# baryshnikova-lab/safepy

Hardware: AMD Instinct MI355X
Metric: node-attribute enrichments/sec (nodes x attrs x perms), compute_pvalues permutation test (higher is better)
Workload: dtype u1 (bit-sliced integer counts; f64 outputs)

## Files before the change

### safepy_amd/csrc/attr.hip

```cpp
#include "common.h"

template <typename T>
__device__ __forceinline__ double load_attr(const void *raw, int64_t idx) {
    return static_cast<double>(reinterpret_cast<const T *>(raw)[idx]);
}

template <typename T, int GC>
__global__ __launch_bounds__(256) void k_attr_stats(const void *__restrict__ raw, int64_t n, int64_t m,
                                                    int64_t rs, int64_t cs, unsigned int *__restrict__ row_bits,
                                                    unsigned long long *__restrict__ acc ,
                                                    double *__restrict__ col_sum, unsigned long long *__restrict__ max_abs_bits,
                                                    unsigned int *__restrict__ col_nan, int64_t rows_per_block) {
    extern __shared__ unsigned int s_bits[];
    constexpr int RL = 256 / GC;
    const int cx = GC == 1 ? 0 : (threadIdx.x & (GC - 1));
    const int ry = GC == 1 ? threadIdx.x : (threadIdx.x / GC);
    const int lane = threadIdx.x & 63;
    const int64_t j = static_cast<int64_t>(blockIdx.x) * GC + cx;
    const int64_t n_words = (n + 31) / 32;
    __shared__ double s_sum[256];
    __shared__ double s_max[256];
    __shared__ unsigned int s_nan[256], s_other[256], s_nonint[256];
    const int64_t r_begin = static_cast<int64_t>(blockIdx.y) * rows_per_block;
    const int64_t r_end = r_begin + rows_per_block < n ? r_begin + rows_per_block : n;
    const int64_t w_begin = r_begin >> 5, w_end = (r_end + 31) >> 5;
    for (int64_t w = w_begin + threadIdx.x; w < w_end; w += 256) s_bits[w] = 0;
    __syncthreads();
    unsigned int c_nan = 0, c_other = 0, c_nonint = 0;
    double mx = 0.0, sum = 0.0;
    constexpr int UN = 4;
    const int64_t n_round = r_begin + (r_end - r_begin + UN * RL - 1) / (UN * RL) * (UN * RL);
    if (GC == 1 && rs == 1) {
        struct __attribute__((packed, aligned(sizeof(T)))) Vec { T v[4]; };
        const T *colp = static_cast<const T *>(raw) + j * cs;
        for (int64_t i0 = r_begin + 4 * static_cast<int64_t>(threadIdx.x); i0 < r_end; i0 += UN * 4 * 256) {
            Vec x[UN];
#pragma unroll
            for (int u = 0; u < UN; ++u) {
                const int64_t i = i0 + static_cast<int64_t>(u) * 4 * 256;
                if (i + 4 <= r_end) {
                    x[u] = *reinterpret_cast<const Vec *>(colp + i);
                } else {
#pragma unroll
                    for (int e = 0; e < 4; ++e) x[u].v[e] = i + e < r_end ? colp[i + e] : static_cast<T>(0);
                }
            }
#pragma unroll
            for (int u = 0; u < UN; ++u) {
                const int64_t i = i0 + static_cast<int64_t>(u) * 4 * 256;
                unsigned int nib = 0;
#pragma unroll
                for (int e = 0; e < 4; ++e) {
                    if (i + e >= r_end) continue;
                    const double v = static_cast<double>(x[u].v[e]);
                    if (v != v) {
                        ++c_nan;
                    } else {
                        nib |= 1u << e;
                        sum += v;
                        if (v != 0.0 && v != 1.0) ++c_other;
                        if (v != floor(v)) ++c_nonint;
                        const double a = fabs(v);
                        if (a > mx) mx = a;
                    }
                }
                if (nib) atomicOr(&s_bits[i >> 5], nib << (i & 31));
            }
        }
    } else
    for (int64_t i0 = r_begin + ry; i0 < n_round; i0 += UN * RL) {
        double v[UN];
        bool inb[UN];
#pragma unroll
        for (int u = 0; u < UN; ++u) {
            const int64_t i = i0 + u * RL;
            inb[u] = i < r_end && j < m;
            v[u] = inb[u] ? load_attr<T>(raw, i * rs + j * cs) : 0.0;
        }
#pragma unroll
        for (int u = 0; u < UN; ++u) {
            const int64_t i = i0 + u * RL;
            bool has = false;
            if (inb[u]) {
                if (v[u] != v[u]) {
                    ++c_nan;
                } else {
                    has = true;
                    sum += v[u];
                    if (v[u] != 0.0 && v[u] != 1.0) ++c_other;
                    if (v[u] != floor(v[u])) ++c_nonint;
                    const double a = fabs(v[u]);
                    if (a > mx) mx = a;
                }
            }
            const unsigned long long bal = __ballot(has);
            if (GC == 1) {
                const int64_t r0 = i - lane;
                if (lane == 0 && bal) {
                    if (r0 < r_end) s_bits[r0 >> 5] |= static_cast<unsigned int>(bal);
                    if (r0 + 32 < r_end) s_bits[(r0 >> 5) + 1] |= static_cast<unsigned int>(bal >> 32);
                }
            } else {
                if (lane == 0 && bal && i < r_end) atomicOr(&s_bits[i >> 5], 1u << (i & 31));
            }
        }
    }
    if (GC == 1) {
        for (int off = 32; off; off >>= 1) {
            sum += __shfl_down(sum, off);
            const double o = __shfl_down(mx, off);
            mx = o > mx ? o : mx;
            c_nan += __shfl_down(c_nan, off);
            c_other += __shfl_down(c_other, off);
            c_nonint += __shfl_down(c_nonint, off);
        }
    }
    const int slot = GC == 1 ? (lane == 0 ? static_cast<int>(threadIdx.x >> 6) : -1) : static_cast<int>(threadIdx.x);
    if (slot >= 0) {
        s_sum[slot] = sum;
        s_max[slot] = mx;
        s_nan[slot] = c_nan;
        s_other[slot] = c_other;
        s_nonint[slot] = c_nonint;
    }
    __syncthreads();
    for (int64_t w = w_begin + threadIdx.x; w < w_end; w += 256) {
        const unsigned int mine = s_bits[w];
        if (mine & ~row_bits[w]) atomicOr(&row_bits[w], mine);
    }
    if (ry == 0 && j < m) {
        double total = 0.0, tmx = 0.0;
        unsigned long long t_nan = 0, t_other = 0, t_nonint = 0;
        for (int r = 0; r < (GC == 1 ? 4 : RL); ++r) {
            const int t = GC == 1 ? r : r * GC + cx;
            total += s_sum[t];
            if (s_max[t] > tmx) tmx = s_max[t];
            t_nan += s_nan[t];
            t_other += s_other[t];
            t_nonint += s_nonint[t];
        }
        if (gridDim.y == 1) col_sum[j] = total;
        else atomicAdd(&col_sum[j], total);
        if (t_nan) atomicAdd(&col_nan[j], static_cast<unsigned int>(t_nan));
        if (t_other) atomicAdd(&acc[4 + (j & 63)], t_other);
        if (t_nonint) atomicAdd(&acc[68 + (j & 63)], t_nonint);
        const unsigned long long mine = static_cast<unsigned long long>(__double_as_longlong(tmx));
        if (mine > __builtin_nontemporal_load(max_abs_bits)) atomicMax(max_abs_bits, mine);
    }
}

__global__ __launch_bounds__(256) void k_stats_finish(unsigned long long *__restrict__ acc, const unsigned int *__restrict__ col_nan, int64_t m,
                                                      const unsigned int *__restrict__ bits, int64_t n, uint8_t *__restrict__ bytes,
                                                      unsigned long long *__restrict__ tail) {
    __shared__ unsigned int s_mx[4];
    __shared__ unsigned long long s_fold[2];
    unsigned int mx = 0;
    for (int64_t i = threadIdx.x; i < m; i += 256) mx = col_nan[i] > mx ? col_nan[i] : mx;
    for (int off = 32; off; off >>= 1) {
        const unsigned int o = __shfl_down(mx, off);
        mx = o > mx ? o : mx;
    }
    if ((threadIdx.x & 63) == 0) s_mx[threadIdx.x >> 6] = mx;
    if (threadIdx.x < 64) {
        unsigned long long a = acc[4 + threadIdx.x], b = acc[68 + threadIdx.x];
        for (int off = 32; off; off >>= 1) {
            a += __shfl_down(a, off);
            b += __shfl_down(b, off);
        }
        if (threadIdx.x == 0) s_fold[0] = a, s_fold[1] = b;
    }
    for (int64_t i = threadIdx.x; i < n; i += 256) bytes[i] = (bits[i >> 5] >> (i & 31)) & 1u;
    __syncthreads();
    if (threadIdx.x == 0) {
        const unsigned int m01 = s_mx[0] > s_mx[1] ? s_mx[0] : s_mx[1], m23 = s_mx[2] > s_mx[3] ? s_mx[2] : s_mx[3];
        tail[0] = acc[0] = s_fold[0];
        tail[1] = acc[1] = m01 > m23 ? m01 : m23;
        tail[2] = acc[2] = s_fold[1];
        tail[3] = acc[3];
    }
}

template <typename T>
__global__ __launch_bounds__(256) void k_fill_support(const void *__restrict__ raw, int64_t n, int64_t m, int64_t rs,
                                                      int64_t cs, const int32_t *__restrict__ sup_ptr,
                                                      int32_t *__restrict__ sup_row) {
    const int64_t j = (static_cast<int64_t>(blockIdx.x) * 256 + threadIdx.x) >> 6;
    const int lane = threadIdx.x & 63;
// ... 99 lines not shown
    SAFE_TRY(dev_alloc(&attr->sup_row, total));
    SAFE_HIP_CHECK(hipMemcpyAsync(attr->sup_ptr, attr->h_sup_ptr.data(), (m + 1) * sizeof(int32_t), hipMemcpyHostToDevice,
                                  ctx->stream));
    if (attr->dtype == SAFE_DTYPE_F32)
        hipLaunchKernelGGL(k_fill_support<float>, dim3(ceil_div(m * 64, 256)), dim3(256), 0, ctx->stream, attr->raw, n, m,
                           attr->row_stride, attr->col_stride, attr->sup_ptr, attr->sup_row);
    else
        hipLaunchKernelGGL(k_fill_support<double>, dim3(ceil_div(m * 64, 256)), dim3(256), 0, ctx->stream, attr->raw, n, m,
                           attr->row_stride, attr->col_stride, attr->sup_ptr, attr->sup_row);
    SAFE_HIP_CHECK(hipGetLastError());
    return SAFE_OK;
}

static size_t flags_block_bytes(int64_t n) { return static_cast<size_t>(ceil_div(n, 8)) * 8 + 32; }

int safe_attr_prepare(safe_attr *attr) {
    if (attr->stats_ready) return SAFE_OK;
    safe_ctx *ctx = attr->ctx;
    SAFE_HIP_CHECK(hipSetDevice(ctx->device));
    const int64_t n = attr->n, m = attr->m;
    const size_t flag_bytes = flags_block_bytes(n), tail_off = flag_bytes - 32;
    const int64_t n_words = (n + 31) / 32;
    SAFE_REQUIRE(n_words * sizeof(unsigned int) <= 150 * 1024, "safe_attr_stats: too many rows for the LDS row bitmap");
    void *tmp = nullptr;
    const size_t tmp_bytes = 132 * sizeof(unsigned long long) + static_cast<size_t>(n_words + m) * sizeof(unsigned int);
    SAFE_TRY(ctx_scratch(ctx, SCRATCH_ATTR_STATS, tmp_bytes, &tmp));
    unsigned long long *d_acc = static_cast<unsigned long long *>(tmp);
    unsigned int *d_rowbits = reinterpret_cast<unsigned int *>(d_acc + 132);
    unsigned int *d_colnan = d_rowbits + n_words;
    SAFE_HIP_CHECK(hipMemsetAsync(tmp, 0, tmp_bytes, ctx->stream));
    uint8_t *flags = nullptr;
    SAFE_TRY(ctx_block_alloc(ctx, flag_bytes, reinterpret_cast<void **>(&flags)));
    if (!attr->col_sum) SAFE_TRY(ctx_block_alloc(ctx, static_cast<size_t>(m) * sizeof(double), reinterpret_cast<void **>(&attr->col_sum)));
    const bool f32 = attr->dtype == SAFE_DTYPE_F32;
    const bool c_order = attr->col_stride == 1 && m > 1;
    if (c_order) SAFE_HIP_CHECK(hipMemsetAsync(attr->col_sum, 0, m * sizeof(double), ctx->stream));
#define STATS(T, GC, RPB)                                                                                          \
    do {                                                                                                           \
        if (n_words * sizeof(unsigned int) > 32 * 1024)                                                            \
            SAFE_HIP_CHECK(hipFuncSetAttribute(reinterpret_cast<const void *>(k_attr_stats<T, GC>),                \
                                               hipFuncAttributeMaxDynamicSharedMemorySize,                         \
                                               static_cast<int>(n_words * sizeof(unsigned int))));                 \
        hipLaunchKernelGGL((k_attr_stats<T, GC>), dim3(ceil_div(m, GC), ceil_div(n, RPB)), dim3(256),              \
                           n_words * sizeof(unsigned int), ctx->stream, attr->raw, n, m, attr->row_stride,         \
                           attr->col_stride, d_rowbits, d_acc, attr->col_sum, d_acc + 3, d_colnan,                 \
                           static_cast<int64_t>(RPB));                                                             \
    } while (0)
    if (c_order) {
        const int64_t groups = ceil_div(m, 64);
        const int64_t want_chunks = std::max<int64_t>(1, 2048 / groups);
        const int64_t rpb = std::max<int64_t>(256, ceil_div(ceil_div(n, want_chunks), 64) * 64);
        if (f32) STATS(float, 64, rpb);
        else STATS(double, 64, rpb);
    } else {
        if (f32) STATS(float, 1, n);
        else STATS(double, 1, n);
    }
#undef STATS
    hipLaunchKernelGGL(k_stats_finish, dim3(1), dim3(256), 0, ctx->stream, d_acc, d_colnan, m, d_rowbits, n, flags,
                       reinterpret_cast<unsigned long long *>(flags + tail_off));
    SAFE_HIP_CHECK(hipGetLastError());
    void *pinned = nullptr;
    SAFE_TRY(ctx_pinned(ctx, flag_bytes, &pinned));
    SAFE_HIP_CHECK(hipMemcpyAsync(pinned, flags, flag_bytes, hipMemcpyDeviceToHost, ctx->stream));
    SAFE_HIP_CHECK(safe_stream_sync(ctx->stream));
    const uint8_t *h_flags = static_cast<const uint8_t *>(pinned);
    unsigned long long h_acc[4];
    memcpy(h_acc, h_flags + tail_off, sizeof(h_acc));
    attr->n_other = static_cast<int64_t>(h_acc[0]);
    attr->max_nan_col = static_cast<int64_t>(h_acc[1]);
    attr->n_non_integer = static_cast<int64_t>(h_acc[2]);
    double mx;
    memcpy(&mx, &h_acc[3], sizeof(double));
    attr->max_abs = mx;
    if (!attr->flags_ready) {
        if (attr->row_flags) ctx_block_free(ctx, attr->row_flags, flag_bytes);
        attr->row_flags = flags;
        attr->flags_ready = true;
        int64_t cnt = 0;
        for (int64_t i = 0; i < n; ++i) cnt += h_flags[i] != 0;
        attr->n_rows_with_value = cnt;
        attr->h_row_flags.assign(h_flags, h_flags + n);
    } else {
        ctx_block_free(ctx, flags, flag_bytes);
    }
    attr->stats_ready = true;
    return SAFE_OK;
}

enum : unsigned int {
    CSC_PTR_FIRST = 1u,
    CSC_PTR_LAST = 2u,
    CSC_PTR_DECREASES = 4u,
    CSC_ROW_EQUAL = 8u,
    CSC_ROW_DESCENDS = 16u,
    CSC_ROW_RANGE = 32u,
    CSC_RULES = 63u,
    CSC_NOT_ONE = 256u,
    CSC_ON_MISSING = 512u,
};

template <typename T>
__global__ __launch_bounds__(256) void k_csc_validate(int64_t n, int64_t m, int64_t nnz, const int64_t *__restrict__ indptr,
                                                      const int32_t *__restrict__ indices, const T *__restrict__ values,
                                                      const uint8_t *__restrict__ missing, int32_t *__restrict__ sup_ptr,
                                                      unsigned int *__restrict__ flag) {
    const int64_t t = static_cast<int64_t>(blockIdx.x) * 256 + threadIdx.x;
    unsigned int bad = 0;
    if (t < nnz) {
        const int32_t r = indices[t];
        if (r < 0 || r >= n) bad |= CSC_ROW_RANGE;
// ... 414 lines not shown
```

### safepy_amd/csrc/common.h

```cpp
#pragma once
#include <hip/hip_runtime.h>

#include <algorithm>
#include <cstdarg>
#include <cmath>
#include <cstdint>
#include <cstdio>
#include <cstdlib>
#include <cstring>
#include <condition_variable>
#include <memory>
#include <mutex>
#include <atomic>
#include <string>
#include <thread>
#include <vector>

#include "safe_hip.h"
#include "bits_plan.h"

#define SAFE_WAVE 64
#define SAFE_PAD_U16 0xFFFFu

void safe_set_error(const char *fmt, ...);
// ... 232 lines not shown
    ~CallTimer() {
        for (hipEvent_t e : ev)
            if (e) (void)hipEventDestroy(e);
    }
    hipError_t start(hipStream_t s) {
        for (hipEvent_t &e : ev) {
            const hipError_t err = hipEventCreateWithFlags(&e, safe_event_flags(hipEventDefault));
            if (err != hipSuccess) return err;
        }
        return hipEventRecord(ev[0], s);
    }
    hipError_t stop(hipStream_t s) { return hipEventRecord(ev[1], s); }
    hipError_t ms(double *out) {
        float f = 0;
        const hipError_t err = hipEventElapsedTime(&f, ev[0], ev[1]);
        *out = f;
        return err;
    }
    hipError_t finish(safe_ctx *ctx, const char *name, int64_t launches, double *kernel_ms) {
        double t = 0;
        const hipError_t err = ms(&t);
        if (err != hipSuccess) return err;
        ctx->last_kernel.name = name;
        ctx->last_kernel.total_ms = ctx->last_kernel.busy_ms = t;
        ctx->last_kernel.launches = launches;
        ctx->last_kernel.summed = true;
        if (kernel_ms) *kernel_ms = t;
        return hipSuccess;
    }
};

struct safe_nbr {
    safe_ctx *ctx = nullptr;
    int64_t n = 0;
    int64_t nnz = 0;
    int64_t max_count = 0;
    int64_t words = 0;
    uint64_t *bits = nullptr;
    int32_t *row_ptr = nullptr;
    int32_t *col = nullptr;
    int64_t n_slices = 0;
    int32_t *sell_row = nullptr;
    int32_t *sell_pos = nullptr;
    int64_t *slice_off = nullptr;
    int32_t *slice_width = nullptr;
    int32_t *sell_col = nullptr;
    int64_t sell_entries = 0;
    uint16_t *sell_col2 = nullptr;
    uint16_t *sell_col2b = nullptr;
    std::vector<int32_t> h_slice_width;
    BitsTaskPlan bits_plan;
    void *bits_plan_pinned = nullptr;
    size_t bits_plan_pinned_bytes = 0;
    std::vector<int64_t> h_slice_off;
    std::vector<int32_t> h_row_count;
    double *dist = nullptr;
    int32_t *at_ptr = nullptr;
    int32_t *at_col = nullptr;
    std::vector<double> h_xy;
    bool blocks_ready = false;
    int64_t bs_groups = 0;
    int64_t bs_blocks = 0;
    int64_t bs_pieces = 0;
    int64_t bs_src = 0;
    int32_t *bs_order = nullptr;
    int32_t *bs_rowmap = nullptr;
    int32_t *bs_rowcnt = nullptr;
    int32_t *bs_grpmax = nullptr;
    uint4 *bs_bits4p = nullptr;
    int64_t bs_max_group_blocks = 0;
    int32_t *bs_ptr = nullptr;
    int32_t *bs_kb = nullptr;
    uint32_t *bs_bits = nullptr;
    std::vector<int32_t> h_bs_ptr;
    std::vector<int32_t> h_bs_rowmap;
    std::vector<int2> counts_tasks;
    int32_t counts_qoff[9] = {0};
    int64_t counts_tasks_grp = -1;
};

struct HypLookup {
    const int32_t *nid;
    const int32_t *kid;
    const double2 *tab;
    int64_t n_kid, xs;
    double p_cut;
    double *dummy;
    double *pvalues_pos, *nes, *nes_binary;
    unsigned int *enriched;
    unsigned int *cnt16;
    unsigned int *xmax;
    int dbg = 0;
};

static inline double nes_p_cut(double enrichment_threshold) {
    const double thr = -std::log10(enrichment_threshold);
    auto hit = [&](double p) { return -std::log10(p) > thr; };
    double p = enrichment_threshold;
    for (int it = 0; it < 4096 && hit(p); ++it) p = std::nextafter(p, 1.0);
    for (int it = 0; it < 4096 && !hit(std::nextafter(p, 0.0)); ++it) p = std::nextafter(p, 0.0);
    return p;
}

enum PermMode {
    PERM_SCORE = 0,
    PERM_COUNTS = 1,
// ... 147 lines not shown
```

### safepy_amd/csrc/enrich.hip

```cpp
#include <algorithm>
#include <cmath>
#include <numeric>

#include "common.h"
#include "hyp_math.h"

template <typename T, int BN, int PLANES>
__global__ __launch_bounds__(256) void k_tile_prep(const void *__restrict__ raw, int64_t n, int64_t rs, int64_t cs,
                                                   int64_t col0, int64_t mloc, int64_t n_tiles,
                                                   double *__restrict__ bt) {
    const int64_t idx = static_cast<int64_t>(blockIdx.x) * 256 + threadIdx.x;
    const int64_t total = n_tiles * (n + 1) * BN;
    if (idx >= total) return;
    const int c = static_cast<int>(idx % BN);
    const int64_t row = (idx / BN) % (n + 1);
    const int64_t tile = idx / (static_cast<int64_t>(BN) * (n + 1));
    const int64_t j = tile * BN + c;
    double v = 0.0, v2 = 0.0, nn = 0.0;
    if (row < n && j < mloc) {
        const T x = reinterpret_cast<const T *>(raw)[row * rs + (col0 + j) * cs];
        if (x == x) {
            v = static_cast<double>(x);
            v2 = static_cast<double>(static_cast<T>(x * x));
            nn = 1.0;
// ... 1116 lines not shown
            }
        } else {
            for (int p = 0; p < np; ++p) {
                uint32_t s0[LV], s1[LV];
#pragma unroll
                for (int l = 0; l < LV; ++l) s0[l] = s1[l] = 0;
                add_pairs(s0, s1);
                settle(p, s0, s1);
            }
        }
    } else {
        for (int p = 0; p < np; ++p, perm_ids += perm_stride) {
            uint32_t s0[LV], s1[LV];
            if (single) {
#pragma unroll
                for (int l = 0; l < LV; ++l) s0[l] = s1[l] = 0;
                const u32x4 *ahead = perm_ids + (p + 2 < np ? 2 * perm_stride : 0) + lane;
                if (p & 1) blk_add8<LV, 0, GATHER>(cb, ahead, s0, s1);
                else blk_add8<LV, 0, GATHER>(ca, ahead, s0, s1);
            } else
                blk_sum<LV, 0, GATHER, (DBG & 32) == 0>(perm_ids, lane, nblk, s0, s1);
            settle(p, s0, s1);
        }
    }
    vflush<CL>(g0, gp0);
    vflush<CL>(g1, gp1);
    vflush<CL>(l0, lp0);
    vflush<CL>(l1, lp1);
    if (STREAM) asm volatile("s_waitcnt vmcnt(0)" : : : "v112", "v113", "v114", "v115", "v116", "v117", "v118", "v119");
}
#pragma clang diagnostic pop

template <int LV, int CL, int DBG>
__device__ __forceinline__ void blk_task(const uint32_t *__restrict__ obs, const u32x4 *__restrict__ perm_ids, int64_t perm_stride,
                                         int lane, int nblk, int np, uint32_t (&g0)[CL], uint32_t (&g1)[CL], uint32_t (&l0)[CL],
                                         uint32_t (&l1)[CL]) {
    blk_task_core<LV, CL, DBG>(obs, perm_ids, perm_stride, lane, nblk, np, g0, g1, l0, l1);
}

template <int LV>
__device__ __forceinline__ void observed_wave(const u32x4 *__restrict__ ids, int lane, int nblk, uint32_t *__restrict__ obs,
                                              uint32_t (&oo0)[BT_LV], uint32_t (&oo1)[BT_LV]) {
    uint32_t o0[LV], o1[LV];
    blk_sum<LV, 2, 1>(ids, lane, nblk, o0, o1);
#pragma unroll
    for (int l = 0; l < BT_LV; ++l) {
        oo0[l] = l < LV ? o0[l < LV ? l : 0] : 0u;
        oo1[l] = l < LV ? o1[l < LV ? l : 0] : 0u;
        obs[l * 64 + lane] = oo0[l];
        obs[(BT_LV + l) * 64 + lane] = oo1[l];
    }
}

__global__ __launch_bounds__(256) void k_bits_observed(int64_t n, const int32_t *__restrict__ sell_row,
                                                       const int64_t *__restrict__ slice_off,
                                                       const int32_t *__restrict__ slice_width,
                                                       const uint16_t *__restrict__ sell_col2b, int64_t n_slices,
                                                       const uint2 *__restrict__ bbits, int64_t mloc,
                                                       uint32_t *__restrict__ obs, double *__restrict__ ns_out) {
    extern __shared__ unsigned int lds[];
    uint2 *T = reinterpret_cast<uint2 *>(lds);
    if ((uint32_t)(uintptr_t)((__attribute__((address_space(3))) unsigned int *)lds) != 0u) __builtin_trap();
    const int wave = __builtin_amdgcn_readfirstlane(threadIdx.x >> 6), lane = threadIdx.x & 63;
    const int64_t wg = blockIdx.x, s = static_cast<int64_t>(blockIdx.y) * 4 + wave;
    load_word_column(T, bbits + wg * (n + 1), n);
    __syncthreads();
    if (s >= n_slices) return;
    const int wdt = __builtin_amdgcn_readfirstlane(slice_width[s]);
    const u32x4 *ids = reinterpret_cast<const u32x4 *>(sell_col2b) + slice_off[s] / 8;
    uint32_t *my_obs = obs + (wg * n_slices + s) * (2 * BT_LV * 64);
    uint32_t oo0[BT_LV], oo1[BT_LV];
    if (wdt <= 8) observed_wave<4>(ids, lane, wdt >> 3, my_obs, oo0, oo1);
    else if (wdt <= 56) observed_wave<6>(ids, lane, wdt >> 3, my_obs, oo0, oo1);
    else if (wdt <= 248) observed_wave<8>(ids, lane, wdt >> 3, my_obs, oo0, oo1);
    else if (wdt <= 504) observed_wave<9>(ids, lane, wdt >> 3, my_obs, oo0, oo1);
    else observed_wave<BT_LV>(ids, lane, wdt >> 3, my_obs, oo0, oo1);
    if (ns_out) {
        const int32_t row = sell_row[s * 64 + lane];
        uint16_t *tile = reinterpret_cast<uint16_t *>(lds + 2 * ((n + 2) & ~int64_t(1)) + 4) + wave * (64 * 66);
#pragma unroll
        for (int half = 0; half < 2; ++half)
#pragma unroll
            for (int bit = 0; bit < 32; ++bit)
                tile[lane * 66 + half * 32 + bit] = static_cast<uint16_t>(half ? vextract<BT_LV>(oo1, bit) : vextract<BT_LV>(oo0, bit));
        const int64_t jc = wg * 64 + lane;
#pragma unroll 8
        for (int r = 0; r < 64; ++r) {
            const int32_t row_r = __shfl(row, r);
            if (row_r >= 0 && jc < mloc) ns_out[static_cast<int64_t>(row_r) * mloc + jc] = static_cast<double>(tile[r * 66 + lane]);
        }
    }
}

template <int CL, bool PLAIN_STORE = false>
__device__ __forceinline__ void flush_counters(const uint32_t (&g0)[CL], const uint32_t (&g1)[CL], const uint32_t (&l0)[CL],
                                               const uint32_t (&l1)[CL], unsigned int *__restrict__ gl_counts, int64_t col0,
                                               int64_t mloc, int64_t n_pad, int64_t spos, bool active) {
#pragma unroll
    for (int half = 0; half < 2; ++half) {
        uint32_t m[32];
#pragma unroll
        for (int l = 0; l < 16; ++l) {
            m[l] = l < CL ? (half ? g1[l < CL ? l : 0] : g0[l < CL ? l : 0]) : 0u;
            m[16 + l] = l < CL ? (half ? l1[l < CL ? l : 0] : l0[l < CL ? l : 0]) : 0u;
        }
        transpose32(m);
        const int64_t c_first = col0 + half * 32;
        const int n_valid = static_cast<int>(mloc - c_first < 32 ? (mloc - c_first > 0 ? mloc - c_first : 0) : 32);
        int64_t off = c_first * n_pad + spos;
#pragma unroll
        for (int bit = 0; bit < 32; ++bit) {
            asm volatile("" : "+v"(off));
            if (PLAIN_STORE) {
                if (bit < n_valid && active && m[bit]) gl_counts[off] = m[bit];
            } else if (bit < n_valid && active && m[bit]) atomicAdd(gl_counts + off, m[bit]);
            off += n_pad;
        }
    }
}

constexpr int BLK_TRACE_MAX = 1 << 17;
__device__ unsigned long long g_blk_trace[BLK_TRACE_MAX * 8];
__device__ unsigned int g_blk_trace_n;

template <int CL, int DBG>
__device__ __forceinline__ void bits_blk_body(

    int64_t n, const uint16_t *__restrict__ ids_p, int64_t entries_pad, const int32_t *__restrict__ sell_row,
    const int64_t *__restrict__ slice_off, const int32_t *__restrict__ slice_width,
    const uint32_t *__restrict__ obs, int64_t n_slices, const uint2 *__restrict__ bbits, BitsQueues qs,
    const int4 *__restrict__ tasks, int64_t p_base, int64_t p_limit, unsigned int *__restrict__ queue, int64_t mloc,
    unsigned int *__restrict__ gl_counts, int64_t n_pad) {
    extern __shared__ unsigned int lds[];
    const int64_t t_words = 2 * ((n + 2) & ~int64_t(1));
    uint2 *T = reinterpret_cast<uint2 *>(lds);
    int *slot_box = reinterpret_cast<int *>(lds + t_words);
    if ((uint32_t)(uintptr_t)((__attribute__((address_space(3))) unsigned int *)lds) != 0u) __builtin_trap();
    const int wave = __builtin_amdgcn_readfirstlane(threadIdx.x >> 6), lane = threadIdx.x & 63;
    const int home = blockIdx.x & 7;
    int tried = 0;

    for (;;) {
        if (threadIdx.x == 0) {
// ... 822 lines not shown
        sw.dbg = 256;
    }
    return sw;
}

static const void *bits_form_kernel(const BitsForm &form, int dbg) {
    const void *blk_fn = nullptr;
    switch (dbg) {
#define BITS_BLK_FN(D) case D: blk_fn = reinterpret_cast<const void *>(k_permtest_bits_blk<8, D>); break;
        BITS_BLK_FN(0) BITS_BLK_FN(32) BITS_BLK_FN(128)
        case 256: blk_fn = reinterpret_cast<const void *>(k_permtest_bits_blk_plain<8, 256>); break;
        case 384: blk_fn = reinterpret_cast<const void *>(k_permtest_bits_blk_plain<8, 384>); break;
        BITS_BLK_FN(512) BITS_BLK_FN(640)
#ifdef SAFE_HIP_DIAG
        BITS_BLK_FN(1) BITS_BLK_FN(2) BITS_BLK_FN(4) BITS_BLK_FN(7) BITS_BLK_FN(8) BITS_BLK_FN(16) BITS_BLK_FN(64) BITS_BLK_FN(1024) BITS_BLK_FN(2048)
#endif
#undef BITS_BLK_FN
        default:
            safe_set_error("SAFE_HIP_BITS_DBG=%d is not a variant of this build (correct variants: 0 32 128 256 384 512 640; the "
                           "work-skipping ones 1 2 4 7 8 16 64 need a library built with make DIAG=1)", dbg);
            return nullptr;
    }
    if (dbg & (95 | 1024 | 2048)) safe_warn_diagnostic("SAFE_HIP_BITS_DBG");
    const bool lv11 = form.levels > BT_LV;
    return form.kind == BITS_BLK ? blk_fn
           : form.half           ? (lv11 ? reinterpret_cast<const void *>(k_permtest_bits_pre32<8, 16, BT_LV + 1>)
                                         : reinterpret_cast<const void *>(k_permtest_bits_pre32<8, 16, BT_LV>))
                                 : (lv11 ? reinterpret_cast<const void *>(k_permtest_bits_pre<BT_LV + 1>)
                                         : reinterpret_cast<const void *>(k_permtest_bits_pre<BT_LV>));
}

static int bits_task_plan(safe_ctx *ctx, safe_nbr *nbr, const BitsForm &form, const BitsTail &tail, const std::vector<int64_t> &starts,
                          int64_t slots, int64_t mloc) {
    const int64_t n_wg = ceil_div(mloc, 64);
    std::vector<int64_t> plan_key = {n_wg, slots, tail.n_major + tail.n_chunks, tail.n_major, tail.n_chunks, tail.wpc, form.waves, form.half ? 1 : 0, mloc};
    plan_key.insert(plan_key.end(), starts.begin(), starts.end());
    BitsTaskPlan &plan = nbr->bits_plan;
    if (plan.key == plan_key) return SAFE_OK;
    plan_bits_tasks(plan, nbr->h_slice_width, nbr->n_slices, form.waves, slots, starts, form.half ? 2 * n_wg : n_wg, mloc, form.half,
                    tail.n_major, tail.n_chunks, tail.wpc);
    const size_t bytes = plan.tasks.size() * sizeof(int4);
    if (nbr->bits_plan_pinned_bytes < bytes) {
        SAFE_HIP_CHECK(safe_stream_sync(ctx->stream));
        if (nbr->bits_plan_pinned) SAFE_HIP_CHECK(hipHostFree(nbr->bits_plan_pinned));
        nbr->bits_plan_pinned = nullptr;
        nbr->bits_plan_pinned_bytes = 0;
        g_alloc_calls.fetch_add(1, std::memory_order_relaxed);
        SAFE_HIP_CHECK(hipHostMalloc(&nbr->bits_plan_pinned, bytes + 4096, hipHostMallocDefault));
        nbr->bits_plan_pinned_bytes = bytes + 4096;
    } else {
        SAFE_HIP_CHECK(safe_stream_sync(ctx->stream));
    }
    memcpy(nbr->bits_plan_pinned, plan.tasks.data(), bytes);
    plan.key = plan_key;
    return SAFE_OK;
}

constexpr int BITS_NS = 2;

struct BitsBuffers {
    uint2 *d_bits = nullptr;
    int4 *d_tasks = nullptr;
    unsigned int *d_queue = nullptr, *d_gl = nullptr;
    int64_t n_pad = 0, entries_pad = 0;
    uint16_t *d_ids[BITS_NS] = {nullptr, nullptr};
    uint16_t *d_ids_tail = nullptr;
    uint32_t *d_obs = nullptr;
};
static int bits_call_buffers(safe_ctx *ctx, const safe_nbr *nbr, const BitsTail &tail, int64_t mloc, int64_t span, int64_t tail_span,
                             BitsBuffers *b) {
    const size_t n_task = nbr->bits_plan.tasks.size();
    const int64_t n_launch = tail.n_major + tail.n_chunks;
    void *ws = nullptr;
    SAFE_TRY(ctx_scratch(ctx, SCRATCH_TASKS, n_task * sizeof(int4) + (8 * n_launch + 4) * sizeof(unsigned int), &ws));
    b->d_tasks = static_cast<int4 *>(ws);
    b->d_queue = reinterpret_cast<unsigned int *>(b->d_tasks + n_task);
    b->n_pad = nbr->n_slices * 64;
    SAFE_TRY(ctx_scratch(ctx, SCRATCH_COUNTERS, static_cast<size_t>(b->n_pad) * mloc * sizeof(unsigned int), reinterpret_cast<void **>(&b->d_gl)));
    SAFE_HIP_CHECK(hipMemcpyAsync(b->d_tasks, nbr->bits_plan_pinned, n_task * sizeof(int4), hipMemcpyHostToDevice, ctx->stream));
    SAFE_HIP_CHECK(hipMemsetAsync(b->d_queue, 0, 8 * n_launch * sizeof(unsigned int), ctx->stream));
    SAFE_HIP_CHECK(hipMemsetAsync(b->d_gl, 0, static_cast<size_t>(b->n_pad) * mloc * sizeof(unsigned int), ctx->stream));
    safe_trace("launch_bits: buffers ready");
    b->entries_pad = (nbr->sell_entries + 1024 + 255) / 256 * 256;
    for (int s = 0; s < BITS_NS; ++s)
        SAFE_TRY(ctx_scratch(ctx, scratch_pair(SCRATCH_STREAM_A, s), static_cast<size_t>(span) * b->entries_pad * sizeof(uint16_t), reinterpret_cast<void **>(&b->d_ids[s])));
    if (tail.n_chunks)
        SAFE_TRY(ctx_scratch(ctx, SCRATCH_BITS_TAIL_IDS, static_cast<size_t>(tail_span) * b->entries_pad * sizeof(uint16_t), reinterpret_cast<void **>(&b->d_ids_tail)));
    return SAFE_OK;
}

static int bits_observe(safe_ctx *ctx, const safe_nbr *nbr, const BitsForm &form, int64_t mloc, double *ns_out, BitsBuffers *b) {
    const int64_t n_wg = ceil_div(mloc, 64);
    SAFE_TRY(ctx_scratch(ctx, SCRATCH_BITS_OBSERVED, static_cast<size_t>(n_wg) * nbr->n_slices * 2 * BT_LV * 64 * sizeof(uint32_t),
                         reinterpret_cast<void **>(&b->d_obs)));
    const size_t lds_obs = form.lds_bytes + (ns_out ? 4 * 64 * 66 * sizeof(uint16_t) : 0);
    SAFE_HIP_CHECK(hipFuncSetAttribute(reinterpret_cast<const void *>(k_bits_observed), hipFuncAttributeMaxDynamicSharedMemorySize,
                                       static_cast<int>(lds_obs)));
    hipLaunchKernelGGL(k_bits_observed, dim3(n_wg, ceil_div(nbr->n_slices, 4)), dim3(256), lds_obs, ctx->stream, nbr->n, nbr->sell_row,
                       nbr->slice_off, nbr->slice_width, nbr->sell_col2b, nbr->n_slices, b->d_bits, mloc, b->d_obs, ns_out);
    SAFE_HIP_CHECK(hipGetLastError());
    return SAFE_OK;
}

static int bits_tail_lists(safe_ctx *ctx, const safe_nbr *nbr, safe_perms *perms, const std::vector<int64_t> &starts, const BitsTail &tail,
                           const BitsBuffers &b, hipEvent_t *plain) {
    hipStream_t tail_ps = ctx->more_streams[1], kstreams[BITS_NS] = {ctx->stream, ctx->side_stream};
    const int64_t n_stage = static_cast<int64_t>(starts.size()) - 1, entries_pad = b.entries_pad;
    SAFE_HIP_CHECK(hipStreamWaitEvent(tail_ps, plain[0], 0));
    for (int64_t t = tail.n_major; t < n_stage; ++t) {
        SAFE_TRY(perms_wait(perms, starts[t + 1], tail_ps));
        hipLaunchKernelGGL(k_permute_cols, dim3(ceil_div(entries_pad, 4096), starts[t + 1] - starts[t]), dim3(256),
                           static_cast<size_t>(perms->stride16) * sizeof(uint16_t), tail_ps, perms->table16, perms->stride16,
                           nbr->sell_col2b, nbr->sell_entries, entries_pad, starts[t], starts[t + 1] - starts[t],
                           static_cast<uint32_t>(8 * nbr->n), b.d_ids_tail + (starts[t] - tail.p_split) * entries_pad, 3);
        SAFE_HIP_CHECK(hipGetLastError());
    }
    SAFE_HIP_CHECK(hipEventRecord(plain[8], tail_ps));
    for (int s = 0; s < BITS_NS; ++s) {
        SAFE_HIP_CHECK(hipEventRecord(plain[4 + s], kstreams[s]));
        SAFE_HIP_CHECK(hipStreamWaitEvent(kstreams[s], plain[8], 0));
    }
    return SAFE_OK;
}

static int bits_launch_spans(safe_ctx *ctx, const safe_nbr *nbr, safe_perms *perms, const BitsForm &form, const void *kfn,
                             const std::vector<int64_t> &starts, const BitsTail &tail, const BitsBuffers &b, int64_t mloc, double *ns_out,
                             const SpanFrame &fr, int *xc_rc) {
    const BitsTaskPlan &plan = nbr->bits_plan;
    const bool blk = form.kind == BITS_BLK;
    const int64_t n = nbr->n, P = perms->count, entries_pad = b.entries_pad, n_pad = b.n_pad;
    hipStream_t kstreams[BITS_NS] = {ctx->stream, ctx->side_stream};
    const int spare = std::min(16, ctx->num_cu / 8);
    const int64_t grid_max = static_cast<int64_t>(std::max(1, ctx->num_cu - spare)) * form.wgs_per_cu;
    auto chunk_final = [&](int64_t c, hipStream_t ks) {
        for (int s = 0; s < BITS_NS; ++s)
            if (kstreams[s] != ks && hipStreamWaitEvent(ks, fr.plain[4 + s], 0) != hipSuccess) *xc_rc = SAFE_E_HIP;
        if (hipEventRecord(ctx->xc_events[c - tail.n_major], ks) != hipSuccess) *xc_rc = SAFE_E_HIP;
    };
    for (int64_t c = 0; c < fr.n_launch; ++c) {
        const bool in_tail = c >= tail.n_major;
        const int64_t p_base = in_tail ? tail.p_split : starts[c], p_limit = in_tail ? P : starts[c + 1];
        const int64_t list = plan.launch_list[c], n_tasks = plan.list_count[list];
        const int4 *d_tasks = b.d_tasks + plan.list_first[list];
        hipStream_t ks = kstreams[c % BITS_NS];
        if (c == tail.n_major) SAFE_TRY(bits_tail_lists(ctx, nbr, perms, starts, tail, b, fr.plain));
        if (!in_tail) SAFE_TRY(perms_wait(perms, p_limit, ks));
        safe_trace("launch_bits: span tables enqueued");
        if (!in_tail)
// ... 829 lines not shown
```

### safepy_amd/csrc/nbr.hip

```cpp
#include <algorithm>
#include <cmath>
#include <numeric>

#include "common.h"

static double squared_threshold(double nr) {
    if (!(nr > 0.0)) return 0.0;
    if (std::isinf(nr)) return nr;
    double c = nr * nr;
    if (std::isinf(c)) return c;
    while (c > 0.0 && std::sqrt(c) >= nr) c = std::nextafter(c, 0.0);
    while (std::sqrt(c) < nr) c = std::nextafter(c, INFINITY);
    return c;
}

__global__ __launch_bounds__(256) void k_euclid_bits(const double *__restrict__ xy, int64_t n, double thr_sq,
                                                     uint64_t *__restrict__ bits, int64_t words) {
    __shared__ double sx[64], sy[64];
    const int64_t w = blockIdx.x;
    const int64_t i = static_cast<int64_t>(blockIdx.y) * 256 + threadIdx.x;
    const int64_t j0 = w * 64;
    if (threadIdx.x < 64) {
        const int64_t j = j0 + threadIdx.x;
        sx[threadIdx.x] = j < n ? xy[2 * j] : 0.0;
// ... 409 lines not shown
            const int used = static_cast<int>(std::min<size_t>(SEL_SLOTS, distinct.size() - g));
            SelPass ps;
            for (int q = 0; q < SEL_SLOTS; ++q) ps.pre[q] = q < used ? distinct[g + q] : ~0ull;
            ps.shift = kSelShift[pass];
            ps.hshift = kSelShift[pass] + kSelBits[pass];
            ps.mask = static_cast<unsigned int>(bins - 1);
            SAFE_TRY(sel_pass(ctx, src, ps, d_hist, h_hist));
            if (pass == 0) {
                unsigned long long total = 0;
                for (int d = 0; d < bins; ++d) total += h_hist[d];
                *count = static_cast<int64_t>(total);
                break;
            }
            for (int64_t t = 0; t < n_ranks; ++t) {
                int q = 0;
                while (q < used && ps.pre[q] != pre[t]) ++q;
                if (q == used) continue;
                const unsigned long long *h = &h_hist[static_cast<size_t>(q) * SEL_BINS];
                int d = 0;
                while (d < bins && static_cast<unsigned long long>(rem[t]) >= h[d]) rem[t] -= static_cast<int64_t>(h[d++]);
                if (d == bins) {
                    safe_set_error("%s: the histograms of pass %d do not hold rank %lld", who, pass, (long long)ranks[t]);
                    return SAFE_E_HIP;
                }
                next[t] = (pre[t] << kSelBits[pass]) | static_cast<unsigned long long>(d);
            }
        }
        if (pass == 0) {
            for (int64_t t = 0; t < n_ranks; ++t) {
                SAFE_REQUIRE(ranks[t] >= 0 && ranks[t] < *count, "%s: rank %lld is outside [0, %lld)", who, (long long)ranks[t],
                             (long long)*count);
                int d = 0;
                while (static_cast<unsigned long long>(rem[t]) >= h_hist[d]) rem[t] -= static_cast<int64_t>(h_hist[d++]);
                next[t] = static_cast<unsigned long long>(d);
            }
            if (n_ranks == 0) return SAFE_OK;
        }
        pre.swap(next);
    }
    SAFE_REQUIRE(src.n >= 2 || n_ranks == 0, "%s: rank %lld is outside [0, 0): one node has no pair", who, (long long)ranks[0]);
    *keys = pre;
    return SAFE_OK;
}

static void nbr_free(safe_nbr *nbr) {
    if (!nbr) return;
    for (const void *q : {(const void *)nbr->bits, (const void *)nbr->row_ptr, (const void *)nbr->col, (const void *)nbr->sell_row,
                          (const void *)nbr->sell_pos, (const void *)nbr->slice_off, (const void *)nbr->slice_width,
                          (const void *)nbr->sell_col, (const void *)nbr->sell_col2, (const void *)nbr->sell_col2b,
                          (const void *)nbr->dist, (const void *)nbr->at_ptr, (const void *)nbr->at_col})
        (void)dev_free(q);
    nbr_free_blocks(nbr);
    if (nbr->bits_plan_pinned) (void)hipHostFree(nbr->bits_plan_pinned);
    delete nbr;
}

using NbrPtr = std::unique_ptr<safe_nbr, void (*)(safe_nbr *)>;

static int nbr_new(safe_ctx *ctx, int64_t n, NbrPtr *out) {
    SAFE_REQUIRE(n >= 1 && n < (1ll << 31) - 64, "neighborhood size n=%lld out of range", (long long)n);
    NbrPtr nbr(new safe_nbr(), nbr_free);
    nbr->ctx = ctx;
    nbr->n = n;
    nbr->words = ceil_div(n, 64);
    SAFE_TRY(dev_alloc(&nbr->bits, static_cast<size_t>(n) * nbr->words));
    *out = std::move(nbr);
    return SAFE_OK;
}

static int nbr_row_counts(safe_nbr *nbr) {
    safe_ctx *ctx = nbr->ctx;
    const int64_t n = nbr->n;
    CallBufs b;
    int32_t *d_count = nullptr;
    SAFE_TRY(b.alloc(&d_count, n));
    hipLaunchKernelGGL(k_row_popcount, dim3(ceil_div(n * 64, 256)), dim3(256), 0, ctx->stream, nbr->bits, n,
                       nbr->words, d_count);
    nbr->h_row_count.resize(n);
    SAFE_HIP_CHECK(hipMemcpyAsync(nbr->h_row_count.data(), d_count, n * sizeof(int32_t), hipMemcpyDeviceToHost,
                                  ctx->stream));
    SAFE_HIP_CHECK(safe_stream_sync(ctx->stream));
    return SAFE_OK;
}

int nbr_finalize_from_bits(safe_nbr *nbr) {
    safe_ctx *ctx = nbr->ctx;
    const int64_t n = nbr->n;
    SAFE_TRY(nbr_row_counts(nbr));

    std::vector<int32_t> row_ptr(n + 1, 0);
    int64_t nnz = 0, max_count = 0;
    for (int64_t i = 0; i < n; ++i) {
        nnz += nbr->h_row_count[i];
        max_count = std::max<int64_t>(max_count, nbr->h_row_count[i]);
        SAFE_REQUIRE(nnz < (1ll << 31), "membership has too many entries for int32 CSR offsets");
        row_ptr[i + 1] = static_cast<int32_t>(nnz);
    }
    nbr->nnz = nnz;
    nbr->max_count = max_count;

    std::vector<int32_t> order(n);
    std::iota(order.begin(), order.end(), 0);
    std::stable_sort(order.begin(), order.end(), [&](int32_t a, int32_t b) {
        return nbr->h_row_count[a] > nbr->h_row_count[b];
    });
    nbr->n_slices = ceil_div(n, 64);
// ... 398 lines not shown
```

Baseline: 6519 billion.

## Add column-chunked attr stats kernel, cache task plan on device, reuse LDS in observed

Adds a new column-major attribute-statistics kernel that splits columns into row chunks spread over waves, doing NaN, other and nonint checks in the native type with nibble popcounts, and removes the old GC==1 path. The bit task plan is now uploaded once to a persistent device buffer when the plan is built, so each launch no longer copies it from host. k_bits_observed gets launch bounds of 4 and reuses its LDS for a packed 32-bit transpose tile instead of appending a separate tile. This adds a sync at plan build and extra code paths whose chunking heuristic may not suit every shape.

```diff
diff --git a/safepy_amd/csrc/attr.hip b/safepy_amd/csrc/attr.hip
--- a/safepy_amd/csrc/attr.hip
+++ b/safepy_amd/csrc/attr.hip
@@ -3,6 +3,122 @@
 template <typename T>
 __device__ __forceinline__ double load_attr(const void *raw, int64_t idx) {
     return static_cast<double>(reinterpret_cast<const T *>(raw)[idx]);
+}
+
+
+template <typename T>
+__global__ __launch_bounds__(256) void k_attr_stats_cols(const T *__restrict__ raw, int64_t n, int64_t m, int64_t cs,
+                                                         int64_t rows_per_unit, int64_t chunks, int64_t units_per_wg,
+                                                         unsigned int *__restrict__ row_bits,
+                                                         unsigned long long *__restrict__ acc ,
+                                                         double *__restrict__ col_sum, unsigned long long *__restrict__ max_abs_bits,
+                                                         unsigned int *__restrict__ col_nan) {
+    extern __shared__ unsigned int s_bits[];
+    __shared__ double s_max[4];
+    __shared__ unsigned int s_other[4], s_nonint[4];
+    const int wave = threadIdx.x >> 6, lane = threadIdx.x & 63;
+    const int64_t n_units = m * chunks;
+    const int64_t u_begin = static_cast<int64_t>(blockIdx.x) * units_per_wg;
+    const int64_t u_end = u_begin + units_per_wg < n_units ? u_begin + units_per_wg : n_units;
+    int64_t r_lo = 0, r_hi = n;
+    if (u_begin / chunks == (u_end - 1) / chunks) {
+        r_lo = (u_begin % chunks) * rows_per_unit;
+        r_hi = ((u_end - 1) % chunks + 1) * rows_per_unit;
+        r_hi = r_hi < n ? r_hi : n;
+    }
+    const int64_t w_lo = r_lo >> 5, w_hi = (r_hi + 31) >> 5;
+    for (int64_t w = w_lo + threadIdx.x; w < w_hi; w += 256) s_bits[w] = 0;
+    __syncthreads();
+    struct __attribute__((packed, aligned(sizeof(T)))) Vec { T v[4]; };
+    constexpr int UN = 32 / sizeof(T);
+    unsigned int c_other = 0, c_nonint = 0;
+    T mx = static_cast<T>(0);
+    for (int64_t u = u_begin + wave; u < u_end; u += 4) {
+        const int64_t j = u / chunks, r_begin = (u - j * chunks) * rows_per_unit;
+        const int64_t r_end = r_begin + rows_per_unit < n ? r_begin + rows_per_unit : n;
+        const T *colp = raw + j * cs;
+        unsigned int c_nan = 0;
+        double sum = 0.0;
+        for (int64_t i0 = r_begin + 4 * lane; i0 < r_end; i0 += UN * 256) {
+            Vec x[UN];
+#pragma unroll
+            for (int k = 0; k < UN; ++k) {
+                const int64_t i = i0 + k * 256;
+                if (i + 4 <= r_end) {
+                    x[k] = *reinterpret_cast<const Vec *>(colp + i);
+                } else {
+#pragma unroll
+                    for (int e = 0; e < 4; ++e) x[k].v[e] = i + e < r_end ? colp[i + e] : static_cast<T>(0);
+                }
+            }
+#pragma unroll
+            for (int k = 0; k < UN; ++k) {
+                const int64_t i = i0 + k * 256;
+                const int left = static_cast<int>(r_end - i < 4 ? (r_end - i > 0 ? r_end - i : 0) : 4);
+                unsigned int nan_nib = 0, other_nib = 0;
+#pragma unroll
+                for (int e = 0; e < 4; ++e) {
+                    const T v = x[k].v[e];
+                    const bool is_nan = v != v;
+                    nan_nib |= static_cast<unsigned int>(is_nan) << e;
+                    other_nib |= static_cast<unsigned int>(!is_nan && v != static_cast<T>(0) && v != static_cast<T>(1)) << e;
+                    sum += static_cast<double>(is_nan ? static_cast<T>(0) : v);
+                    mx = fmax(mx, fabs(v));
+                }
+                c_nan += __popc(nan_nib);
+                if (other_nib) {
+                    c_other += __popc(other_nib);
+#pragma unroll
+                    for (int e = 0; e < 4; ++e) c_nonint += ((other_nib >> e) & 1u) && x[k].v[e] != floor(x[k].v[e]);
+                }
+                const unsigned int nib = ~nan_nib & ((1u << left) - 1u);
+                if (nib) atomicOr(&s_bits[i >> 5], nib << (i & 31));
+            }
+        }
+        for (int off = 32; off; off >>= 1) {
+            sum += __shfl_down(sum, off);
+            c_nan += __shfl_down(c_nan, off);
+        }
+        if (lane == 0) {
+            if (chunks == 1) {
+                col_sum[j] = sum;
+                if (c_nan) col_nan[j] = c_nan;
+            } else {
+                atomicAdd(&col_sum[j], sum);
+                if (c_nan) atomicAdd(&col_nan[j], c_nan);
+            }
+        }
+    }
+    for (int off = 32; off; off >>= 1) {
+        c_other += __shfl_down(c_other, off);
+        c_nonint += __shfl_down(c_nonint, off);
+        const T o = __shfl_down(mx, off);
+        mx = o > mx ? o : mx;
+    }
+    if (lane == 0) {
+        s_max[wave] = static_cast<double>(mx);
+        s_other[wave] = c_other;
+        s_nonint[wave] = c_nonint;
+    }
+    __syncthreads();
+    if (wave == 0) {
+        for (int64_t w = w_lo + lane; w < w_hi; w += 64) {
+            const unsigned int mine = s_bits[w];
+            if (mine & ~row_bits[w]) atomicOr(&row_bits[w], mine);
+        }
+    } else if (threadIdx.x == 64) {
+        double tmx = 0.0;
+        unsigned long long t_other = 0, t_nonint = 0;
+        for (int r = 0; r < 4; ++r) {
+            if (s_max[r] > tmx) tmx = s_max[r];
+            t_other += s_other[r];
+            t_nonint += s_nonint[r];
+        }
+        if (t_other) atomicAdd(&acc[4 + (blockIdx.x & 63)], t_other);
+        if (t_nonint) atomicAdd(&acc[68 + (blockIdx.x & 63)], t_nonint);
+        const unsigned long long mine = static_cast<unsigned long long>(__double_as_longlong(tmx));
+        if (mine > __builtin_nontemporal_load(max_abs_bits)) atomicMax(max_abs_bits, mine);
+    }
 }
 
 template <typename T, int GC>
@@ -13,11 +129,10 @@
                                                     unsigned int *__restrict__ col_nan, int64_t rows_per_block) {
     extern __shared__ unsigned int s_bits[];
     constexpr int RL = 256 / GC;
-    const int cx = GC == 1 ? 0 : (threadIdx.x & (GC - 1));
-    const int ry = GC == 1 ? threadIdx.x : (threadIdx.x / GC);
+    const int cx = threadIdx.x & (GC - 1);
+    const int ry = threadIdx.x / GC;
     const int lane = threadIdx.x & 63;
     const int64_t j = static_cast<int64_t>(blockIdx.x) * GC + cx;
-    const int64_t n_words = (n + 31) / 32;
     __shared__ double s_sum[256];
     __shared__ double s_max[256];
     __shared__ unsigned int s_nan[256], s_other[256], s_nonint[256];
@@ -30,44 +145,6 @@
     double mx = 0.0, sum = 0.0;
     constexpr int UN = 4;
     const int64_t n_round = r_begin + (r_end - r_begin + UN * RL - 1) / (UN * RL) * (UN * RL);
-    if (GC == 1 && rs == 1) {
-        struct __attribute__((packed, aligned(sizeof(T)))) Vec { T v[4]; };
-        const T *colp = static_cast<const T *>(raw) + j * cs;
-        for (int64_t i0 = r_begin + 4 * static_cast<int64_t>(threadIdx.x); i0 < r_end; i0 += UN * 4 * 256) {
-            Vec x[UN];
-#pragma unroll
-            for (int u = 0; u < UN; ++u) {
-                const int64_t i = i0 + static_cast<int64_t>(u) * 4 * 256;
-                if (i + 4 <= r_end) {
-                    x[u] = *reinterpret_cast<const Vec *>(colp + i);
-                } else {
-#pragma unroll
-                    for (int e = 0; e < 4; ++e) x[u].v[e] = i + e < r_end ? colp[i + e] : static_cast<T>(0);
-                }
-            }
-#pragma unroll
-            for (int u = 0; u < UN; ++u) {
-                const int64_t i = i0 + static_cast<int64_t>(u) * 4 * 256;
-                unsigned int nib = 0;
-#pragma unroll
-                for (int e = 0; e < 4; ++e) {
-                    if (i + e >= r_end) continue;
-                    const double v = static_cast<double>(x[u].v[e]);
-                    if (v != v) {
-                        ++c_nan;
-                    } else {
-                        nib |= 1u << e;
-                        sum += v;
-                        if (v != 0.0 && v != 1.0) ++c_other;
-                        if (v != floor(v)) ++c_nonint;
-                        const double a = fabs(v);
-                        if (a > mx) mx = a;
-                    }
-                }
-                if (nib) atomicOr(&s_bits[i >> 5], nib << (i & 31));
-            }
-        }
-    } else
     for (int64_t i0 = r_begin + ry; i0 < n_round; i0 += UN * RL) {
         double v[UN];
         bool inb[UN];
@@ -94,35 +171,14 @@
                 }
             }
             const unsigned long long bal = __ballot(has);
-            if (GC == 1) {
-                const int64_t r0 = i - lane;
-                if (lane == 0 && bal) {
-                    if (r0 < r_end) s_bits[r0 >> 5] |= static_cast<unsigned int>(bal);
-                    if (r0 + 32 < r_end) s_bits[(r0 >> 5) + 1] |= static_cast<unsigned int>(bal >> 32);
-                }
-            } else {
-                if (lane == 0 && bal && i < r_end) atomicOr(&s_bits[i >> 5], 1u << (i & 31));
-            }
-        }
-    }
-    if (GC == 1) {
-        for (int off = 32; off; off >>= 1) {
-            sum += __shfl_down(sum, off);
-            const double o = __shfl_down(mx, off);
-            mx = o > mx ? o : mx;
-            c_nan += __shfl_down(c_nan, off);
-            c_other += __shfl_down(c_other, off);
-            c_nonint += __shfl_down(c_nonint, off);
-        }
-    }
-    const int slot = GC == 1 ? (lane == 0 ? static_cast<int>(threadIdx.x >> 6) : -1) : static_cast<int>(threadIdx.x);
-    if (slot >= 0) {
-        s_sum[slot] = sum;
-        s_max[slot] = mx;
-        s_nan[slot] = c_nan;
-        s_other[slot] = c_other;
-        s_nonint[slot] = c_nonint;
-    }
+            if (lane == 0 && bal && i < r_end) atomicOr(&s_bits[i >> 5], 1u << (i & 31));
+        }
+    }
+    s_sum[threadIdx.x] = sum;
+    s_max[threadIdx.x] = mx;
+    s_nan[threadIdx.x] = c_nan;
+    s_other[threadIdx.x] = c_other;
+    s_nonint[threadIdx.x] = c_nonint;
     __syncthreads();
     for (int64_t w = w_begin + threadIdx.x; w < w_end; w += 256) {
         const unsigned int mine = s_bits[w];
@@ -131,8 +187,8 @@
     if (ry == 0 && j < m) {
         double total = 0.0, tmx = 0.0;
         unsigned long long t_nan = 0, t_other = 0, t_nonint = 0;
-        for (int r = 0; r < (GC == 1 ? 4 : RL); ++r) {
-            const int t = GC == 1 ? r : r * GC + cx;
+        for (int r = 0; r < RL; ++r) {
+            const int t = r * GC + cx;
             total += s_sum[t];
             if (s_max[t] > tmx) tmx = s_max[t];
             t_nan += s_nan[t];
@@ -338,11 +394,33 @@
         const int64_t rpb = std::max<int64_t>(256, ceil_div(ceil_div(n, want_chunks), 64) * 64);
         if (f32) STATS(float, 64, rpb);
         else STATS(double, 64, rpb);
-    } else {
-        if (f32) STATS(float, 1, n);
-        else STATS(double, 1, n);
     }
 #undef STATS
+#define STATS_COLS(T)                                                                                              \
+    do {                                                                                                           \
+        if (n_words * sizeof(unsigned int) > 32 * 1024)                                                            \
+            SAFE_HIP_CHECK(hipFuncSetAttribute(reinterpret_cast<const void *>(k_attr_stats_cols<T>),               \
+                                               hipFuncAttributeMaxDynamicSharedMemorySize,                         \
+                                               static_cast<int>(n_words * sizeof(unsigned int))));                 \
+        hipLaunchKernelGGL((k_attr_stats_cols<T>), dim3(ceil_div(units, units_per_wg)), dim3(256),                 \
+                           n_words * sizeof(unsigned int), ctx->stream, static_cast<const T *>(attr->raw), n, m,   \
+                           attr->col_stride, rows_per_unit, chunks, units_per_wg, d_rowbits, d_acc, attr->col_sum, \
+                           d_acc + 3, d_colnan);                                                                   \
+    } while (0)
+    if (!c_order) {
+        const int64_t wave_slots = 16 * static_cast<int64_t>(ctx->num_cu);
+        int64_t chunks = 1, rows_per_unit = n;
+        if (m < wave_slots && n > 4096) {
+            const int64_t want = std::min(ceil_div(n, 4096), ceil_div(wave_slots, m));
+            rows_per_unit = ceil_div(ceil_div(n, want), 2048) * 2048;
+            chunks = ceil_div(n, rows_per_unit);
+        }
+        const int64_t units = m * chunks, units_per_wg = 4 * ceil_div(units, 2 * wave_slots);
+        if (chunks > 1) SAFE_HIP_CHECK(hipMemsetAsync(attr->col_sum, 0, m * sizeof(double), ctx->stream));
+        if (f32) STATS_COLS(float);
+        else STATS_COLS(double);
+    }
+#undef STATS_COLS
     hipLaunchKernelGGL(k_stats_finish, dim3(1), dim3(256), 0, ctx->stream, d_acc, d_colnan, m, d_rowbits, n, flags,
                        reinterpret_cast<unsigned long long *>(flags + tail_off));
     SAFE_HIP_CHECK(hipGetLastError());
diff --git a/safepy_amd/csrc/common.h b/safepy_amd/csrc/common.h
--- a/safepy_amd/csrc/common.h
+++ b/safepy_amd/csrc/common.h
@@ -308,6 +308,8 @@
     BitsTaskPlan bits_plan;
     void *bits_plan_pinned = nullptr;
     size_t bits_plan_pinned_bytes = 0;
+    void *bits_plan_dev = nullptr;
+    size_t bits_plan_dev_bytes = 0;
     std::vector<int64_t> h_slice_off;
     std::vector<int32_t> h_row_count;
     double *dist = nullptr;
diff --git a/safepy_amd/csrc/enrich.hip b/safepy_amd/csrc/enrich.hip
--- a/safepy_amd/csrc/enrich.hip
+++ b/safepy_amd/csrc/enrich.hip
@@ -1192,12 +1192,12 @@
     }
 }
 
-__global__ __launch_bounds__(256) void k_bits_observed(int64_t n, const int32_t *__restrict__ sell_row,
-                                                       const int64_t *__restrict__ slice_off,
-                                                       const int32_t *__restrict__ slice_width,
-                                                       const uint16_t *__restrict__ sell_col2b, int64_t n_slices,
-                                                       const uint2 *__restrict__ bbits, int64_t mloc,
-                                                       uint32_t *__restrict__ obs, double *__restrict__ ns_out) {
+__global__ __launch_bounds__(256, 4) void k_bits_observed(int64_t n, const int32_t *__restrict__ sell_row,
+                                                          const int64_t *__restrict__ slice_off,
+                                                          const int32_t *__restrict__ slice_width,
+                                                          const uint16_t *__restrict__ sell_col2b, int64_t n_slices,
+                                                          const uint2 *__restrict__ bbits, int64_t mloc,
+                                                          uint32_t *__restrict__ obs, double *__restrict__ ns_out) {
     extern __shared__ unsigned int lds[];
     uint2 *T = reinterpret_cast<uint2 *>(lds);
     if ((uint32_t)(uintptr_t)((__attribute__((address_space(3))) unsigned int *)lds) != 0u) __builtin_trap();
@@ -1205,30 +1205,39 @@
     const int64_t wg = blockIdx.x, s = static_cast<int64_t>(blockIdx.y) * 4 + wave;
     load_word_column(T, bbits + wg * (n + 1), n);
     __syncthreads();
-    if (s >= n_slices) return;
-    const int wdt = __builtin_amdgcn_readfirstlane(slice_width[s]);
-    const u32x4 *ids = reinterpret_cast<const u32x4 *>(sell_col2b) + slice_off[s] / 8;
-    uint32_t *my_obs = obs + (wg * n_slices + s) * (2 * BT_LV * 64);
+    const bool live = s < n_slices;
     uint32_t oo0[BT_LV], oo1[BT_LV];
-    if (wdt <= 8) observed_wave<4>(ids, lane, wdt >> 3, my_obs, oo0, oo1);
-    else if (wdt <= 56) observed_wave<6>(ids, lane, wdt >> 3, my_obs, oo0, oo1);
-    else if (wdt <= 248) observed_wave<8>(ids, lane, wdt >> 3, my_obs, oo0, oo1);
-    else if (wdt <= 504) observed_wave<9>(ids, lane, wdt >> 3, my_obs, oo0, oo1);
-    else observed_wave<BT_LV>(ids, lane, wdt >> 3, my_obs, oo0, oo1);
-    if (ns_out) {
-        const int32_t row = sell_row[s * 64 + lane];
-        uint16_t *tile = reinterpret_cast<uint16_t *>(lds + 2 * ((n + 2) & ~int64_t(1)) + 4) + wave * (64 * 66);
-#pragma unroll
-        for (int half = 0; half < 2; ++half)
-#pragma unroll
-            for (int bit = 0; bit < 32; ++bit)
-                tile[lane * 66 + half * 32 + bit] = static_cast<uint16_t>(half ? vextract<BT_LV>(oo1, bit) : vextract<BT_LV>(oo0, bit));
-        const int64_t jc = wg * 64 + lane;
+    if (live) {
+        const int wdt = __builtin_amdgcn_readfirstlane(slice_width[s]);
+        const u32x4 *ids = reinterpret_cast<const u32x4 *>(sell_col2b) + slice_off[s] / 8;
+        uint32_t *my_obs = obs + (wg * n_slices + s) * (2 * BT_LV * 64);
+        if (wdt <= 8) observed_wave<4>(ids, lane, wdt >> 3, my_obs, oo0, oo1);
+        else if (wdt <= 56) observed_wave<6>(ids, lane, wdt >> 3, my_obs, oo0, oo1);
+        else if (wdt <= 248) observed_wave<8>(ids, lane, wdt >> 3, my_obs, oo0, oo1);
+        else if (wdt <= 504) observed_wave<9>(ids, lane, wdt >> 3, my_obs, oo0, oo1);
+        else observed_wave<BT_LV>(ids, lane, wdt >> 3, my_obs, oo0, oo1);
+    }
+    if (!ns_out) return;
+    __syncthreads();
+    if (!live) return;
+    const int32_t row = sell_row[s * 64 + lane];
+    uint32_t *tile = lds + wave * (64 * 33);
+#pragma unroll
+    for (int half = 0; half < 2; ++half) {
+#pragma unroll
+        for (int c = 0; c < 32; c += 2) {
+            const uint32_t lo = half ? vextract<BT_LV>(oo1, c) : vextract<BT_LV>(oo0, c);
+            const uint32_t hi = half ? vextract<BT_LV>(oo1, c + 1) : vextract<BT_LV>(oo0, c + 1);
+            tile[lane * 33 + half * 16 + (c >> 1)] = lo | (hi << 16);
+        }
+    }
+    const int64_t jc = wg * 64 + lane;
+    const int pair = lane >> 1, shift = (lane & 1) * 16;
 #pragma unroll 8
-        for (int r = 0; r < 64; ++r) {
-            const int32_t row_r = __shfl(row, r);
-            if (row_r >= 0 && jc < mloc) ns_out[static_cast<int64_t>(row_r) * mloc + jc] = static_cast<double>(tile[r * 66 + lane]);
-        }
+    for (int r = 0; r < 64; ++r) {
+        const int32_t row_r = __shfl(row, r);
+        const uint32_t val = (tile[r * 33 + pair] >> shift) & 0xFFFFu;
+        if (row_r >= 0 && jc < mloc) ns_out[static_cast<int64_t>(row_r) * mloc + jc] = static_cast<double>(val);
     }
 }
 
@@ -2157,6 +2166,15 @@
         SAFE_HIP_CHECK(safe_stream_sync(ctx->stream));
     }
     memcpy(nbr->bits_plan_pinned, plan.tasks.data(), bytes);
+    if (nbr->bits_plan_dev_bytes < bytes) {
+        SAFE_HIP_CHECK(dev_free(nbr->bits_plan_dev));
+        nbr->bits_plan_dev = nullptr;
+        nbr->bits_plan_dev_bytes = 0;
+        SAFE_TRY(dev_alloc_bytes(&nbr->bits_plan_dev, bytes + 4096));
+        nbr->bits_plan_dev_bytes = bytes + 4096;
+    }
+    if (bytes) SAFE_HIP_CHECK(hipMemcpyAsync(nbr->bits_plan_dev, nbr->bits_plan_pinned, bytes, hipMemcpyHostToDevice, ctx->stream));
+    SAFE_HIP_CHECK(safe_stream_sync(ctx->stream));
     plan.key = plan_key;
     return SAFE_OK;
 }
@@ -2177,12 +2195,12 @@
     const size_t n_task = nbr->bits_plan.tasks.size();
     const int64_t n_launch = tail.n_major + tail.n_chunks;
     void *ws = nullptr;
-    SAFE_TRY(ctx_scratch(ctx, SCRATCH_TASKS, n_task * sizeof(int4) + (8 * n_launch + 4) * sizeof(unsigned int), &ws));
-    b->d_tasks = static_cast<int4 *>(ws);
-    b->d_queue = reinterpret_cast<unsigned int *>(b->d_tasks + n_task);
+    SAFE_REQUIRE(n_task * sizeof(int4) <= nbr->bits_plan_dev_bytes, "launch_bits: the task lists are not on the device");
+    SAFE_TRY(ctx_scratch(ctx, SCRATCH_TASKS, (8 * n_launch + 4) * sizeof(unsigned int), &ws));
+    b->d_tasks = static_cast<int4 *>(nbr->bits_plan_dev);
+    b->d_queue = static_cast<unsigned int *>(ws);
     b->n_pad = nbr->n_slices * 64;
     SAFE_TRY(ctx_scratch(ctx, SCRATCH_COUNTERS, static_cast<size_t>(b->n_pad) * mloc * sizeof(unsigned int), reinterpret_cast<void **>(&b->d_gl)));
-    SAFE_HIP_CHECK(hipMemcpyAsync(b->d_tasks, nbr->bits_plan_pinned, n_task * sizeof(int4), hipMemcpyHostToDevice, ctx->stream));
     SAFE_HIP_CHECK(hipMemsetAsync(b->d_queue, 0, 8 * n_launch * sizeof(unsigned int), ctx->stream));
     SAFE_HIP_CHECK(hipMemsetAsync(b->d_gl, 0, static_cast<size_t>(b->n_pad) * mloc * sizeof(unsigned int), ctx->stream));
     safe_trace("launch_bits: buffers ready");
@@ -2198,7 +2216,7 @@
     const int64_t n_wg = ceil_div(mloc, 64);
     SAFE_TRY(ctx_scratch(ctx, SCRATCH_BITS_OBSERVED, static_cast<size_t>(n_wg) * nbr->n_slices * 2 * BT_LV * 64 * sizeof(uint32_t),
                          reinterpret_cast<void **>(&b->d_obs)));
-    const size_t lds_obs = form.lds_bytes + (ns_out ? 4 * 64 * 66 * sizeof(uint16_t) : 0);
+    const size_t lds_obs = std::max<size_t>(form.lds_bytes, ns_out ? 4 * 64 * 33 * sizeof(uint32_t) : 0);
     SAFE_HIP_CHECK(hipFuncSetAttribute(reinterpret_cast<const void *>(k_bits_observed), hipFuncAttributeMaxDynamicSharedMemorySize,
                                        static_cast<int>(lds_obs)));
     hipLaunchKernelGGL(k_bits_observed, dim3(n_wg, ceil_div(nbr->n_slices, 4)), dim3(256), lds_obs, ctx->stream, nbr->n, nbr->sell_row,
diff --git a/safepy_amd/csrc/nbr.hip b/safepy_amd/csrc/nbr.hip
--- a/safepy_amd/csrc/nbr.hip
+++ b/safepy_amd/csrc/nbr.hip
@@ -485,6 +485,7 @@
         (void)dev_free(q);
     nbr_free_blocks(nbr);
     if (nbr->bits_plan_pinned) (void)hipHostFree(nbr->bits_plan_pinned);
+    (void)dev_free(nbr->bits_plan_dev);
     delete nbr;
 }
 
```

After: 6603 billion (median of 6 runs). 1.3% higher.
